# imatge-upc/rsis

Measured on AMD Instinct MI355X. Metric: training images/sec at 256x256, T=10, batch=32 per GPU, higher is better.
Workload: dtype f32

## Files before the change

rsis_amd/csrc/api.hip:

```cpp
#include "common.h"
#include "../../include/rsis_hip.h"
#include "launchers.h"
#include <stdlib.h>

static inline int krows_of(int C, int ks) { return rsis_roundup(C * ks * ks, RSIS_KPAD); }
static inline int log2i(int s) { int l = 0; while ((1 << l) < s) ++l; return l; }
static inline bool use_direct(int ks, int stride, int pad) { return ks == 3 && stride == 1 && pad == 1; }
static inline bool use_direct_s2(int ks, int stride, int pad) { return ks == 3 && stride == 2 && pad == 1; }
static inline bool use_direct_f2(int ks, int stride, int pad) {
  static const bool on = !(getenv("RSIS_CONV_F2") && getenv("RSIS_CONV_F2")[0] == '0');
  return on && use_direct_s2(ks, stride, pad);
}
static inline bool use_direct_fwd(int ks, int stride, int pad) { return use_direct(ks, stride, pad) || use_direct_f2(ks, stride, pad); }
static inline int seg_chunks(int nseg, const int* Cseg, int ck) {
  int q = 0;
  for (int s = 0; s < nseg; ++s) q += (Cseg[s] + ck - 1) / ck;
  return q;
}
static inline int direct_rows(int nseg, const int* Cseg) { return seg_chunks(nseg, Cseg, RSIS_CK) * RSIS_CK * 9; }
static inline bool bf16_geom(int ks, int stride, int pad, int Cout) {
  return Cout > 1 && ((ks == 3 && stride == 1 && pad == 1) || (ks == 1 && pad == 0));
}
static inline bool use_bf16(int dtype, int ks, int stride, int pad, int Cout) {
  return dtype == RSIS_DTYPE_BF16 && bf16_geom(ks, stride, pad, Cout);
}
static inline bool wino_geom(int ks, int stride, int pad, int Cin, int Cout, int nseg, int lstm_hid) {
  return ks == 3 && stride == 1 && pad == 1 && nseg == 1 && lstm_hid == 0 && Cin >= 32 && Cout >= 32 && Cin % 32 == 0 && Cout % 32 == 0;
}
static inline bool wino_geom_dgrad(int ks, int stride, int pad, int Cin, int Cout) {
  return ks == 3 && stride == 1 && pad == 1 && Cin >= 32 && Cout >= 32 && Cin % 32 == 0 && Cout % 32 == 0;
}
static inline bool use_wino(int dtype, int ks, int stride, int pad, int Cin, int Cout, int nseg, int lstm_hid) {
  return dtype == RSIS_DTYPE_F32_WINO && wino_geom(ks, stride, pad, Cin, Cout, nseg, lstm_hid);
}
static inline int bf16_rows(int ks, int nseg, const int* Cseg) {
  const int ckb = bf16_ckb(ks * ks);
  return seg_chunks(nseg, Cseg, ckb) * ks * ks * (ckb / 8);
}
static int g_deterministic = -1;
int rsis_deterministic() {
  if (g_deterministic < 0) g_deterministic = (getenv("RSIS_DETERMINISTIC") && getenv("RSIS_DETERMINISTIC")[0] == '1') ? 1 : 0;
  return g_deterministic;
}
static inline bool conv_splitk_ok() {
  static const bool env_ok = !(getenv("RSIS_CONV_SPLITK") && getenv("RSIS_CONV_SPLITK")[0] == '0');
  return env_ok && !rsis_deterministic();
}
static inline bool splitk_geom(int B, int H, int W, int rows, int nq, int min_chunks) {
  const long px_tiles = (long)B * rsis_cdiv(H, 8) * rsis_cdiv(W, W <= 8 ? 8 : 16);
  return nq >= min_chunks && px_tiles * rsis_cdiv(rows, 64) < 160;
}
static int zero_dsts(const ConvArgs& a, hipStream_t st) {
  for (int i = 0; i < a.ndst; ++i)
    if (rsis_zero_async(a.dst[i], sizeof(float) * (size_t)a.B * a.Cd[i] * a.oH * a.oW, st) != RSIS_OK) return RSIS_ERR_LAUNCH;
  return RSIS_OK;
}
static int splitk_enable(ConvArgs& a, hipStream_t st) { a.ksplit = 0; return zero_dsts(a, st); }
static inline int direct_variant(int tile) { const int v = tile % 10; return (tile > 0 && v >= 1 && v <= 9) ? v : 0; }

extern "C" {

int rsis_version(void) { return RSIS_ABI_VERSION; }

int rsis_set_deterministic(int on) {
// ... 179 lines not shown
  a.nsrc = nsrc;
  a.K = 0;
  for (int s = 0; s < RSIS_MAX_SRC; ++s) { a.src[s] = nsrc > 0 ? src[0] : nullptr; a.C[s] = 0; }
  for (int s = 0; s < nsrc; ++s) {
    if (!src[s] || Csrc[s] < 1) return RSIS_ERR_ARG;
    a.src[s] = src[s]; a.C[s] = Csrc[s]; a.K += Csrc[s] * ks * ks;
  }
  return RSIS_OK;
}

struct BnEval { const float* gamma; const float* beta; const float* mean; const float* var; float eps; int relu; };

static int conv2d_fwd_impl(const float* const* src, const int* Csrc, int nsrc, int B, int H, int W, const void* Wp, int Cout,
                           int ks, int stride, int pad, const float* bias, const float* addend, float* out, int Ho, int Wo,
                           int tile, int dtype, void* stream, const BnEval* bn) {
  const bool allow_splitk = tile >= 100;
  tile %= 100;
  ConvArgs a = {};
  int rc = fill_sources(a, src, Csrc, nsrc, ks);
  if (rc) return rc;
  if (!Wp || !out || B < 1 || stride < 1) return RSIS_ERR_ARG;
  if (Ho != (H + 2 * pad - ks) / stride + 1 || Wo != (W + 2 * pad - ks) / stride + 1) return RSIS_ERR_ARG;
  a.B = B; a.H = H; a.W = W; a.Ho = Ho; a.Wo = Wo; a.stride = stride; a.pad = pad; a.sshift = 0;
  a.wp = (const float*)Wp; a.ldw = rsis_roundup(Cout, RSIS_LDW_ALIGN); a.Cout = Cout; a.bias = bias; a.addend = addend;
  a.dst[0] = out; a.Cd[0] = Cout; a.ndst = 1;
  a.ostride = 1; a.oH = Ho; a.oW = Wo; a.ksplit = 1;
  a.precise = allow_splitk ? 0 : 1;
  if (bn) {
    if (!bn->gamma || !bn->beta || !bn->mean || !bn->var) return RSIS_ERR_ARG;
    if (allow_splitk || Cout % 4 != 0 || (size_t)B * Cout * Ho * Wo * 4 >= (1ull << 31)) return RSIS_ERR_UNSUPPORTED;
    if (dtype != RSIS_DTYPE_F32 && (dtype != RSIS_DTYPE_BF16 || use_bf16(dtype, ks, stride, pad, Cout))) return RSIS_ERR_UNSUPPORTED;
    if (use_direct(ks, stride, pad) && Cout == 1) return RSIS_ERR_UNSUPPORTED;
    a.ep_gamma = bn->gamma; a.ep_beta = bn->beta; a.ep_mean = bn->mean; a.ep_var = bn->var; a.ep_eps = bn->eps; a.ep_relu = bn->relu ? 1 : 0;
  }
  if (use_wino(dtype, ks, stride, pad, Csrc[0], Cout, nsrc, 0))
    return rsis_launch_conv_wino(src[0], Wp, bias, addend, out, B, Csrc[0], Cout, H, W, (hipStream_t)stream, a.precise);
  if (use_bf16(dtype, ks, stride, pad, Cout)) {
    if (stride != 1) return RSIS_ERR_UNSUPPORTED;
    if (ks == 1 && nsrc != 1) return RSIS_ERR_UNSUPPORTED;
    if (ks == 3 && allow_splitk && conv_splitk_ok() && !addend && splitk_geom(B, H, W, Cout, seg_chunks(a.nsrc, a.C, RSIS_CKB3), 16) &&
        splitk_enable(a, (hipStream_t)stream))
      return RSIS_ERR_LAUNCH;
    return rsis_launch_conv_bf16(a, ks, 0, direct_variant(tile), (hipStream_t)stream);
  }
  if (use_direct(ks, stride, pad) && Cout == 1 && nsrc == 1 && !addend && rsis_c1_supported(Csrc[0]) && W % 4 == 0)
    return rsis_l_c1_fwd(src[0], (const float*)Wp, a.ldw, bias, out, B, Csrc[0], H, W, 1, (hipStream_t)stream);
  if (use_direct(ks, stride, pad)) {
    if (allow_splitk && conv_splitk_ok() && splitk_geom(B, H, W, Cout, seg_chunks(a.nsrc, a.C, RSIS_CK), 32) && splitk_enable(a, (hipStream_t)stream))
      return RSIS_ERR_LAUNCH;
    return rsis_launch_conv3x3_direct(a, 0, direct_variant(tile), (hipStream_t)stream);
  }
  if (use_direct_f2(ks, stride, pad))
    return rsis_launch_conv3x3_direct(a, 3, direct_variant(tile), (hipStream_t)stream);
  return rsis_launch_conv_igemm(a, ks, false, 0, tile, (hipStream_t)stream);
}

int rsis_conv2d_fwd(const float* const* src, const int* Csrc, int nsrc, int B, int H, int W, const void* Wp, int Cout,
                    int ks, int stride, int pad, const float* bias, const float* addend, float* out, int Ho, int Wo,
                    int tile, int dtype, void* stream) {
  return conv2d_fwd_impl(src, Csrc, nsrc, B, H, W, Wp, Cout, ks, stride, pad, bias, addend, out, Ho, Wo, tile, dtype, stream, nullptr);
}

int rsis_conv2d_fwd_bn_eval(const float* const* src, const int* Csrc, int nsrc, int B, int H, int W, const void* Wp, int Cout,
                            int ks, int stride, int pad, const float* bias, const float* addend, const float* gamma, const float* beta,
                            const float* running_mean, const float* running_var, float eps, int relu, float* out, int Ho, int Wo,
                            int tile, int dtype, void* stream) {
  const BnEval bn = {gamma, beta, running_mean, running_var, eps, relu};
  return conv2d_fwd_impl(src, Csrc, nsrc, B, H, W, Wp, Cout, ks, stride, pad, bias, addend, out, Ho, Wo, tile % 100, dtype, stream, &bn);
}

static int dgrad_fill(ConvArgs& a, const float* dy, int B, int Cout, int Hy, int Wy, const void* Wd, int Cin_packed, int ks, int stride, int pad,
                      float* const* dx, const int* Cdx, int ndst, int Hx, int Wx, const float* addend) {
  a = ConvArgs{};
  const float* srcs[1] = {dy};
  const int cs[1] = {Cout};
  const int rc = fill_sources(a, srcs, cs, 1, ks);
  if (rc) return rc;
  int ctot = 0;
  for (int i = 0; i < ndst; ++i) { if (!dx[i] || Cdx[i] < 1) return RSIS_ERR_ARG; a.dst[i] = dx[i]; a.Cd[i] = Cdx[i]; ctot += Cdx[i]; }
  if (ctot > Cin_packed) return RSIS_ERR_ARG;
  a.ndst = ndst;
  a.B = B; a.H = Hy; a.W = Wy; a.Ho = Hx; a.Wo = Wx; a.stride = stride; a.pad = pad; a.sshift = log2i(stride);
  a.ostride = 1; a.oH = Hx; a.oW = Wx; a.ksplit = 1;
  a.wp = (const float*)Wd; a.ldw = rsis_roundup(Cin_packed, RSIS_LDW_ALIGN); a.Cout = ctot; a.bias = nullptr; a.addend = addend;
  return RSIS_OK;
}

int rsis_conv2d_dgrad(const float* dy, int B, int Cout, int Hy, int Wy, const void* Wd, int Cin_packed, int ks, int stride,
                      int pad, float* const* dx, const int* Cdx, int ndst, int Hx, int Wx, const float* addend, int tile,
                      int dtype, void* stream) {
  if (!dy || !Wd || !dx || !Cdx || ndst < 1 || ndst > RSIS_MAX_SRC) return RSIS_ERR_ARG;
  const bool inplace = addend && ndst == 1 && stride > 1 && ks == 1 && pad == 0 && addend == dx[0];
  if (addend && !inplace && (ndst != 1 || stride != 1)) return RSIS_ERR_UNSUPPORTED;
  if (stride != 1 && stride != 2 && stride != 4) return RSIS_ERR_UNSUPPORTED;
  ConvArgs a;
  const int rc = dgrad_fill(a, dy, B, Cout, Hy, Wy, Wd, Cin_packed, ks, stride, pad, dx, Cdx, ndst, Hx, Wx, addend);
  if (rc) return rc;
  const int ctot = a.Cout;
  if (dtype == RSIS_DTYPE_F32_WINO && wino_geom_dgrad(ks, stride, pad, Cin_packed, Cout)) {
    if (ndst > 2 || ctot % 32 != 0 || Cdx[0] % 32 != 0 || Hx != Hy || Wx != Wy || (ndst == 2 && addend)) return RSIS_ERR_UNSUPPORTED;
    if (ndst == 1) return rsis_launch_conv_wino(dy, Wd, nullptr, addend, dx[0], B, Cout, ctot, Hy, Wy, (hipStream_t)stream, 0);
    const float* xs[1] = {dy}; const void* us[1] = {Wd}; float* y0[1] = {dx[0]}; float* y1[1] = {dx[1]};
    const int b1[1] = {B}, c1[1] = {Cout}, co1[1] = {ctot}, c01[1] = {Cdx[0]}, h1[1] = {Hy}, w1[1] = {Wy};
    return rsis_launch_conv_wino_group(1, xs, us, y0, y1, b1, c1, co1, c01, h1, w1, (hipStream_t)stream);
  }
  if (use_bf16(dtype, ks, stride, pad, Cout)) {
    if (ks == 3) {
      if (Hx != Hy || Wx != Wy) return RSIS_ERR_ARG;
      if (conv_splitk_ok() && !addend && splitk_geom(B, Hx, Wx, ctot, seg_chunks(a.nsrc, a.C, RSIS_CKB3), 16) && splitk_enable(a, (hipStream_t)stream))
        return RSIS_ERR_LAUNCH;
      return rsis_launch_conv_bf16(a, 3, 0, direct_variant(tile), (hipStream_t)stream);
    }
    if (stride > 1) {
      if (Hy != (Hx - 1) / stride + 1 || Wy != (Wx - 1) / stride + 1) return RSIS_ERR_ARG;
      if (!inplace && zero_dsts(a, (hipStream_t)stream)) return RSIS_ERR_LAUNCH;
      a.ostride = stride;
    } else if (Hx != Hy || Wx != Wy) return RSIS_ERR_ARG;
    a.Ho = Hy; a.Wo = Wy; a.stride = 1; a.sshift = 0;
    return rsis_launch_conv_bf16(a, 1, 0, direct_variant(tile), (hipStream_t)stream);
  }
  if (use_direct(ks, stride, pad)) {
    if (Hx != Hy || Wx != Wy) return RSIS_ERR_ARG;
    if (Cout == 1 && ndst == 1 && Cin_packed == Cdx[0] && rsis_c1_supported(Cdx[0]) && !addend)
      return rsis_l_c1_dgrad(dy, (const float*)Wd, a.ldw, dx[0], B, Cdx[0], Hx, Wx, 1, (hipStream_t)stream);
    if (conv_splitk_ok() && !addend && splitk_geom(B, Hx, Wx, ctot, seg_chunks(a.nsrc, a.C, RSIS_CK), 32) && splitk_enable(a, (hipStream_t)stream))
      return RSIS_ERR_LAUNCH;
    return rsis_launch_conv3x3_direct(a, 0, direct_variant(tile), (hipStream_t)stream);
  }
  if (use_direct_s2(ks, stride, pad) && ndst == 1 && Cdx[0] == Cin_packed && Hy == (Hx + 1) / 2 && Wy == (Wx + 1) / 2) {
    a.Ho = Hy; a.Wo = Wy; a.oH = Hx; a.oW = Wx;
    return rsis_launch_conv3x3_direct(a, 2, direct_variant(tile), (hipStream_t)stream);
  }
  if (ks == 1 && pad == 0 && stride > 1) {
    if (!inplace && zero_dsts(a, (hipStream_t)stream)) return RSIS_ERR_LAUNCH;
    a.Ho = Hy; a.Wo = Wy; a.stride = 1; a.sshift = 0; a.ostride = stride;
    return rsis_launch_conv_igemm(a, ks, false, 0, tile, (hipStream_t)stream);
  }
  return rsis_launch_conv_igemm(a, ks, true, 0, tile, (hipStream_t)stream);
}

static int wgrad_route(WgradArgs& a, int ks, int lstm_hid, int dtype) {
  if (dtype == RSIS_DTYPE_BF16_BLK) {
    a.blk = 1;
    return rsis_wgrad_bf16_supported(a, ks) ? 1 : -1;
  }
  if (use_direct(ks, a.stride, a.pad) && a.Cout == 1 && lstm_hid == 0 && rsis_c1_supported(a.Cs) && a.H == a.Ho && a.W == a.Wo && a.W % 4 == 0)
    return 0;
  if (dtype == RSIS_DTYPE_BF16 && rsis_wgrad_bf16_supported(a, ks)) return 1;
  static const bool tiled_ok = !(getenv("RSIS_WGRAD_TILED") && getenv("RSIS_WGRAD_TILED")[0] == '0');
  if (tiled_ok && rsis_wgrad_tiled_supported(a, ks)) return 2;
  return 3;
}
static int wgrad_fill(WgradArgs& a, const float* dy, const float* x, float* dW, int B, int Cs, int H, int W, int Cout, int Ho, int Wo,
                      int ks, int stride, int pad, int Ctot, int c_off, int lstm_hid) {
  if (!dy || !x || !dW || c_off < 0 || c_off + Cs > Ctot) return RSIS_ERR_ARG;
  a = WgradArgs{};
  a.dy = dy; a.x = x; a.dw = dW; a.B = B; a.Cs = Cs; a.H = H; a.W = W; a.Ho = Ho; a.Wo = Wo; a.Cout = Cout;
  a.stride = stride; a.pad = pad; a.ldo = Ctot * ks * ks; a.n_off = c_off * ks * ks; a.interleave_hid = lstm_hid;
  return RSIS_OK;
}
static int wgrad_launch_one(WgradArgs& a, int route, int ks, hipStream_t st) {
  switch (route) {
    case 0: return rsis_l_c1_wgrad(a.dy, a.x, a.dw + a.n_off, nullptr, a.B, a.Cs, a.H, a.W, 1, st);
    case 1: return rsis_launch_conv_wgrad_bf16(a, ks, st);
    case 2: return rsis_launch_conv_wgrad_tiled(a, ks, st);
    default: return rsis_launch_conv_wgrad(a, ks, st);
  }
}

int rsis_conv2d_wgrad(const float* dy, const float* x, float* dW, int B, int Cs, int H, int W, int Cout, int Ho, int Wo,
                      int ks, int stride, int pad, int Ctot, int c_off, int lstm_hid, int dtype, void* stream) {
  WgradArgs a;
  const int rc = wgrad_fill(a, dy, x, dW, B, Cs, H, W, Cout, Ho, Wo, ks, stride, pad, Ctot, c_off, lstm_hid);
  if (rc) return rc;
  const int route = wgrad_route(a, ks, lstm_hid, dtype);
  if (route < 0) return RSIS_ERR_UNSUPPORTED;
  return wgrad_launch_one(a, route, ks, (hipStream_t)stream);
}

int rsis_conv2d_wgrad_batch(const rsis_wgrad_job* jobs, int njobs, void* stream) {
  if (!jobs || njobs < 1) return RSIS_ERR_ARG;
  WgradArgs* tiled[4] = {(WgradArgs*)malloc(sizeof(WgradArgs) * njobs), (WgradArgs*)malloc(sizeof(WgradArgs) * njobs),
                         (WgradArgs*)malloc(sizeof(WgradArgs) * njobs), (WgradArgs*)malloc(sizeof(WgradArgs) * njobs)};
  int nt[4] = {0, 0, 0, 0};
  int rc = (tiled[0] && tiled[1] && tiled[2] && tiled[3]) ? RSIS_OK : RSIS_ERR_LAUNCH;
  for (int j = 0; j < njobs && rc == RSIS_OK; ++j) {
    const rsis_wgrad_job& q = jobs[j];
    WgradArgs a;
    rc = wgrad_fill(a, q.dy, q.x, q.dW, q.B, q.Cs, q.H, q.W, q.Cout, q.Ho, q.Wo, q.ks, q.stride, q.pad, q.Ctot, q.c_off, q.lstm_hid);
    if (rc) break;
    const int route = wgrad_route(a, q.ks, q.lstm_hid, q.dtype);
    if (route < 0) { rc = RSIS_ERR_UNSUPPORTED; break; }
    if ((route == 1 || route == 2) && (q.ks == 1 || q.ks == 3) && !rsis_deterministic()) {
      const int li = (route == 1 ? 2 : 0) + (q.ks == 3);
      tiled[li][nt[li]++] = a;
    } else rc = wgrad_launch_one(a, route, q.ks, (hipStream_t)stream);
  }
  if (rc == RSIS_OK) rc = rsis_launch_conv_wgrad_tiled_group(tiled[0], nt[0], 1, (hipStream_t)stream);
  if (rc == RSIS_OK) rc = rsis_launch_conv_wgrad_tiled_group(tiled[1], nt[1], 3, (hipStream_t)stream);
  if (rc == RSIS_OK) rc = rsis_launch_conv_wgrad_bf16_group(tiled[2], nt[2], 1, (hipStream_t)stream);
  if (rc == RSIS_OK) rc = rsis_launch_conv_wgrad_bf16_group(tiled[3], nt[3], 3, (hipStream_t)stream);
  for (int i = 0; i < 4; ++i) free(tiled[i]);
  return rc;
}

int rsis_bias_grad(const float* dy, float* db, int B, int C, int HW, int lstm_hid, void* stream) {
  if (!dy || !db) return RSIS_ERR_ARG;
  return rsis_l_channel_sum(dy, db, B, C, HW, lstm_hid, (hipStream_t)stream);
}

static int lstm_fill(ConvArgs& a, int& route, const float* const* src, const int* Csrc, int nsrc, int B, int H, int W, const void* Wp,
                     const float* bias_packed, const float* addend, const float* c_prev, float* h_out, float* c_out, float* act_out, int hid,
                     int ks, int pad, int dtype, unsigned long long* side_key = nullptr) {
  a = ConvArgs{};
  int rc = fill_sources(a, src, Csrc, nsrc, ks, addend != nullptr);
  if (rc) return rc;
  if (!Wp || !h_out || !c_out || hid < 1 || B < 1) return RSIS_ERR_ARG;
  if (2 * pad != ks - 1) return RSIS_ERR_UNSUPPORTED;
// ... 564 lines not shown
```

rsis_amd/csrc/launchers.h:

```cpp
#pragma once
#include "common.h"
#include "../../include/rsis_hip.h"

int rsis_launch_conv_igemm(ConvArgs& a, int ks, bool dgrad, int epi, int force_tile, hipStream_t st);
int rsis_launch_conv3x3_direct(ConvArgs& a, int epi, int force_variant, hipStream_t st);
int rsis_launch_convlstm_direct_group(ConvArgs* jobs, int n, const int* force_variant, hipStream_t st);
int rsis_launch_conv3x3_direct_group_plain(ConvArgs* jobs, int n, const int* force_variant, hipStream_t st);
int rsis_launch_conv_wino(const float* x, const void* U, const float* bias, const float* addend, float* y, int B, int C, int Cout, int H, int W, hipStream_t st,
                          int precise);
int rsis_launch_conv_wino_group(int n, const float* const* x, const void* const* U, float* const* y, float* const* y1, const int* B, const int* C, const int* Cout,
                                const int* C0, const int* H, const int* W, hipStream_t st);
int rsis_launch_conv_bf16(ConvArgs& a, int ks, int epi, int force_variant, hipStream_t st);
int rsis_launch_conv_blk(ConvArgs& a, int ks, int variant, hipStream_t st);
int rsis_l_blk_from_nchw(const float* x, void* y, int B, int C, int HW, hipStream_t st);
int rsis_l_blk_to_nchw(const void* x, float* y, int B, int C, int HW, hipStream_t st);
int rsis_launch_conv_blk_dec(BlkConvJob* jobs, int n, int epi, const int* force_variant, hipStream_t st);
int rsis_launch_conv_wgrad(WgradArgs& a, int ks, hipStream_t st);
bool rsis_wgrad_bf16_supported(const WgradArgs& w, int ks);
int rsis_launch_conv_wgrad_bf16_group(const WgradArgs* w, int n, int ks, hipStream_t st);
int rsis_launch_conv_wgrad_bf16(const WgradArgs& w, int ks, hipStream_t st);
int rsis_launch_conv_wgrad_tiled_group(const WgradArgs* w, int n, int ks, hipStream_t st);
int rsis_launch_conv_wgrad_tiled(const WgradArgs& w, int ks, hipStream_t st);
bool rsis_wgrad_tiled_supported(const WgradArgs& w, int ks);
bool rsis_c1_supported(int Cin);
int rsis_l_c1_fwd(const float* x, const float* wp, int ldw, const float* bias, float* y, int B, int Cin, int H, int W, int seqT, hipStream_t st);
int rsis_l_c1_dgrad(const float* dy, const float* wd, int ldw, float* dx, int B, int Cin, int H, int W, int seqT, hipStream_t st);
int rsis_l_c1_wgrad(const float* dy, const float* x, float* dw, float* db, int B, int Cin, int H, int W, int seqT, hipStream_t st);
bool rsis_upconv_supported(int C, int Hs, int Ws, int Ho, int Wo);
int rsis_upconv_bwd_blocks(int T, int B, int Hs, int Ws);
int rsis_l_upconv_fwd(const void* h, int h_blk, const float* w, const float* bias, float* out, int T, int B, int Hs, int Ws, int Ho, int Wo, hipStream_t st);
int rsis_l_upconv_bwd(const float* dout, const void* h, int h_blk, const float* w, void* dh, float* dW, float* db, const float* dside, const int* arg,
                      float* partial, int T, int B, int Hs, int Ws, int Ho, int Wo, hipStream_t st);
int rsis_l_pack_batch(const rsis_pack_job* jobs, int njobs, int total_blocks, hipStream_t st);
int rsis_l_pack_blocks(PackMode mode, int krows, int ldw, int ks);
int rsis_l_pack(PackMode mode, const float* W, void* out, int Cout, int Ctot, int ks, int nseg, const int* Cseg, const int* Coff, int ldw, int krows, int hid,
                hipStream_t st);
int rsis_l_lstm_bwd(const float* dh, const float* dh2, const float* dc_next, const float* act, const float* c_prev, const float* c, float* da, float* dc_prev,
                    float* da_sum, int B, int hid, int HW, hipStream_t st);
int rsis_l_lstm_bwd_group(const void* const* ptrs, const int* dims, int n, hipStream_t st);
int rsis_l_upsample_fwd(const float* x, float* y, long BC, int Hi, int Wi, int Ho, int Wo, hipStream_t st);
int rsis_l_upsample_bwd(const float* dy, float* dx, long BC, int Hi, int Wi, int Ho, int Wo, const float* pool_g, const int* pool_arg, hipStream_t st);
int rsis_l_gmax_fwd(const float* x, float* y, int* arg, long BC, int HW, hipStream_t st);
int rsis_l_gmax_bwd(const float* dy, const int* arg, float* dx, long BC, int HW, hipStream_t st);
int rsis_l_bn_fwd(const float* x, const float* res, float* y, unsigned char* mask, double* stats, const float* gamma, const float* beta, float* run_mean,
                  float* run_var, float* save_mean, float* save_rstd, int B, int C, int HW, float eps, float momentum, int relu, int train_flags, hipStream_t st);
int rsis_l_bn_bwd(const float* dy, const float* x, const float* y, const unsigned char* mask, const float* mean, const float* rstd, const float* gamma,
                  double* stats, float* dx, float* dres, float* dgamma, float* dbeta, int B, int C, int HW, int relu_flags, float eval_eps, hipStream_t st);
int rsis_l_gmax_bwd_add(const float* dy, const int* arg, float* dx, long BC, int HW, hipStream_t st);
int rsis_l_subsample(const float* x, float* y, long BC, int H, int W, int Ho, int Wo, int s, hipStream_t st);
int rsis_l_maxpool_fwd(const float* x, float* y, unsigned char* arg, long BC, int H, int W, int Ho, int Wo, hipStream_t st);
int rsis_l_maxpool_bwd(const float* dy, const unsigned char* arg, float* dx, long BC, int H, int W, int Ho, int Wo, int accumulate, hipStream_t st);
int rsis_l_sum_leading(const float* x, float* y, int T, long n, hipStream_t st);
int rsis_l_channel_sum(const float* dy, float* db, int B, int C, int HW, int hid, hipStream_t st);
int rsis_l_adam(float* p, const float* g, float* m, float* v, long n, float lr, float b1, float b2, float eps, float wd, int step, float gscale, const int* step_dev,
                hipStream_t st);
int rsis_l_assign(const float* scores, long long* perm, int B, int G, int T, hipStream_t st);
int rsis_l_flat_rule(int rule, float* p, const float* g, float* s, long n, float lr, float c0, float c1, float wd, float gscale, hipStream_t st);
// ... 64 lines not shown
```

rsis_amd/csrc/pointwise.hip:

```cpp
#include "common.h"
#include "launchers.h"
#include <cstdlib>

__global__ void lstm_bwd_kernel(const float* __restrict__ dh, const float* __restrict__ dh2, const float* __restrict__ dc_next,
                                const float* __restrict__ act, const float* __restrict__ c_prev,
                                const float* __restrict__ c, float* __restrict__ da, float* __restrict__ dc_prev,
                                float* __restrict__ da_sum, int hid, int HW, long total) {
  for (long e = blockIdx.x * (long)blockDim.x + threadIdx.x; e < total; e += (long)gridDim.x * blockDim.x) {
    const long bj = e / HW;
    const int sp = (int)(e - bj * HW);
    const long g0 = bj * 4 * HW + sp;
    const float gi = act[g0], gf = act[g0 + HW], go = act[g0 + 2L * HW], gg = act[g0 + 3L * HW];
    const float tc = tanhf(c[e]);
    const float dhv = (dh ? dh[e] : 0.f) + (dh2 ? dh2[e] : 0.f);
    float dcv = dhv * go * (1.f - tc * tc);
    if (dc_next) dcv += dc_next[e];
    const float cp = c_prev ? c_prev[e] : 0.f;
    const float dai = dcv * gg * gi * (1.f - gi);
    const float daf = dcv * cp * gf * (1.f - gf);
    const float dao = dhv * tc * go * (1.f - go);
    const float dag = dcv * gi * (1.f - gg * gg);
    da[g0] = dai; da[g0 + HW] = daf; da[g0 + 2L * HW] = dao; da[g0 + 3L * HW] = dag;
    if (da_sum) { da_sum[g0] += dai; da_sum[g0 + HW] += daf; da_sum[g0 + 2L * HW] += dao; da_sum[g0 + 3L * HW] += dag; }
    if (dc_prev) dc_prev[e] = dcv * gf;
// ... 661 lines not shown
      const size_t idx = ((size_t)b * C + c) * HW + sp;
      f32x4 o;
#pragma unroll
      for (int k = 0; k < 4; ++k) o[k] = kk * (g[i][k] - mg - xh[i][k] * mgx);
      *reinterpret_cast<f32x4*>(dx + idx) = o;
      if (dres) *reinterpret_cast<f32x4*>(dres + idx) = g[i];
    }
  }
}

__global__ void subsample_kernel(const float* __restrict__ x, float* __restrict__ y, int H, int W, int Ho, int Wo, int s, long total4) {
  const int wq = (Wo + 3) / 4;
  for (long e = blockIdx.x * (long)blockDim.x + threadIdx.x; e < total4; e += (long)gridDim.x * blockDim.x) {
    const int q = (int)(e % wq);
    const long t = e / wq;
    const int ho = (int)(t % Ho);
    const long bc = t / Ho;
    const float* xr = x + (bc * H + (long)ho * s) * W;
    float* yr = y + (bc * Ho + ho) * (long)Wo + 4 * q;
    if (s == 2 && (W & 3) == 0 && 4 * q + 3 < Wo && 8 * q + 7 < W) {
      const f32x4 a = *reinterpret_cast<const f32x4*>(xr + 8 * q), b = *reinterpret_cast<const f32x4*>(xr + 8 * q + 4);
      const f32x4 o = {a[0], a[2], b[0], b[2]};
      if ((Wo & 3) == 0) *reinterpret_cast<f32x4*>(yr) = o;
      else { yr[0] = o[0]; yr[1] = o[1]; yr[2] = o[2]; yr[3] = o[3]; }
    } else {
      for (int k = 0; k < 4 && 4 * q + k < Wo; ++k) yr[k] = xr[(long)(4 * q + k) * s];
    }
  }
}

__global__ void maxpool3x3s2_fwd_kernel(const float* __restrict__ x, float* __restrict__ y, unsigned char* __restrict__ arg,
                                        int H, int W, int Ho, int Wo, long total) {
  for (long e = blockIdx.x * (long)blockDim.x + threadIdx.x; e < total; e += (long)gridDim.x * blockDim.x) {
    const int wo = (int)(e % Wo);
    const long t = e / Wo;
    const int ho = (int)(t % Ho);
    const long bc = t / Ho;
    const float* xb = x + bc * H * W;
    float v[9];
    bool ok[9];
#pragma unroll
    for (int r = 0; r < 3; ++r)
#pragma unroll
      for (int s = 0; s < 3; ++s) {
        const int h = ho * 2 - 1 + r, w = wo * 2 - 1 + s;
        ok[r * 3 + s] = (unsigned)h < (unsigned)H && (unsigned)w < (unsigned)W;
        v[r * 3 + s] = xb[min(max(h, 0), H - 1) * W + min(max(w, 0), W - 1)];
      }
    float best = -INFINITY; int bi = 0;
#pragma unroll
    for (int k = 0; k < 9; ++k)
      if (ok[k] && (v[k] > best || v[k] != v[k])) { best = v[k]; bi = k; }
    y[e] = best; arg[e] = (unsigned char)bi;
  }
}

__global__ void maxpool3x3s2_bwd_kernel(const float* __restrict__ dy, const unsigned char* __restrict__ arg,
                                        float* __restrict__ dx, int H, int W, int Ho, int Wo, long total, int accumulate) {
  for (long e = blockIdx.x * (long)blockDim.x + threadIdx.x; e < total; e += (long)gridDim.x * blockDim.x) {
    const int w = (int)(e % W);
    const long t = e / W;
    const int h = (int)(t % H);
    const long bc = t / H;
    float g = 0.f;
    const int ho_lo = h >> 1, wo_lo = w >> 1;
#pragma unroll
    for (int a = 0; a < 2; ++a) {
#pragma unroll
      for (int b = 0; b < 2; ++b) {
        const int ho = ho_lo + a, wo = wo_lo + b;
        const int r = h - (ho * 2 - 1), s = w - (wo * 2 - 1);
        const bool ok = ho < Ho && r >= 0 && r <= 2 && wo < Wo && s >= 0 && s <= 2;
        const long o = (bc * Ho + min(ho, Ho - 1)) * Wo + min(wo, Wo - 1);
        const int ar = arg[o];
        const float d = dy[o];
        g += (ok && ar == r * 3 + s) ? d : 0.f;
      }
    }
    if (accumulate) g += dx[e];
    dx[e] = g;
  }
}

__global__ __launch_bounds__(256) void maxpool3x3s2_bwd_v8_kernel(const float* __restrict__ dy, const unsigned char* __restrict__ arg,
                                                                  float* __restrict__ dx, int H, int W, int Ho, int Wo, long items,
                                                                  int accumulate) {
  const int Wq = W >> 2, Hp = H >> 1;
  for (long e = blockIdx.x * (long)blockDim.x + threadIdx.x; e < items; e += (long)gridDim.x * blockDim.x) {
    const int wq = (int)(e % Wq);
    const long t = e / Wq;
    const int hp = (int)(t % Hp);
    const long bc = t / Hp;
    const int h0 = hp * 2, w0 = wq * 4;
    float d[6];
    int th[6], tw[6];
#pragma unroll
    for (int a = 0; a < 2; ++a)
#pragma unroll
      for (int b = 0; b < 3; ++b) {
        const int ho = hp + a, wo = wq * 2 + b;
        const bool ok = ho < Ho && wo < Wo;
        const long o = (bc * Ho + min(ho, Ho - 1)) * Wo + min(wo, Wo - 1);
        const int ar = arg[o];
        d[a * 3 + b] = dy[o];
        th[a * 3 + b] = ok ? ho * 2 - 1 + ar / 3 - h0 : -1;
        tw[a * 3 + b] = wo * 2 - 1 + ar % 3 - w0;
// ... 377 lines not shown
}
template <int NT, int VPT>
static void bn_bwd_fused_launch(const float* dy, const float* x, const float* y, const unsigned char* mask, const float* mean,
                                const float* rstd, const float* gamma, float* dx, float* dres, float* dgamma, float* dbeta, int C,
                                int HW, long N, int relu, int accum, hipStream_t st) {
  if (mask)
    hipLaunchKernelGGL((bn_bwd_fused_kernel<NT, VPT, true>), dim3(C), dim3(NT), 0, st, dy, x, y, mask, mean, rstd, gamma, dx, dres,
                       dgamma, dbeta, C, HW, N, relu, accum);
  else
    hipLaunchKernelGGL((bn_bwd_fused_kernel<NT, VPT, false>), dim3(C), dim3(NT), 0, st, dy, x, y, mask, mean, rstd, gamma, dx, dres,
                       dgamma, dbeta, C, HW, N, relu, accum);
}
int rsis_l_bn_bwd(const float* dy, const float* x, const float* y, const unsigned char* mask, const float* mean, const float* rstd,
                  const float* gamma, double* stats, float* dx, float* dres, float* dgamma, float* dbeta, int B, int C, int HW,
                  int relu_flags, float eval_eps, hipStream_t st) {
  const long N = (long)B * HW;
  const int S = chan_splits(C, N);
  const int relu = relu_flags & 1, accum = (relu_flags >> 2) & 1;
  if (mask && (!relu || (HW & 3))) return RSIS_ERR_UNSUPPORTED;
  if (eval_eps < 0.f && bn_fused_ok(C, HW, N)) {
    if (N / 4 <= 256 * 8 && C <= 512)
      bn_bwd_fused_launch<512, 4>(dy, x, y, mask, mean, rstd, gamma, dx, dres, dgamma, dbeta, C, HW, N, relu, accum, st);
    else if (N / 4 <= 256 * 8)
      bn_bwd_fused_launch<256, 8>(dy, x, y, mask, mean, rstd, gamma, dx, dres, dgamma, dbeta, C, HW, N, relu, accum, st);
    else
      bn_bwd_fused_launch<1024, 8>(dy, x, y, mask, mean, rstd, gamma, dx, dres, dgamma, dbeta, C, HW, N, relu, accum, st);
    return rsis_check_launch();
  }
  if (!(relu_flags & 2) && rsis_zero_async(stats, sizeof(double) * 2 * C, st) != RSIS_OK) return RSIS_ERR_LAUNCH;
  if (mask) {
    hipLaunchKernelGGL(bn_bwd_reduce_kernel<true>, dim3(C, S), dim3(256), 0, st, dy, x, y, mask, mean, rstd, stats, C, HW, N, relu,
                       eval_eps);
    hipLaunchKernelGGL(bn_bwd_apply_kernel<true>, dim3(C, S), dim3(256), 0, st, dy, x, y, mask, mean, rstd, gamma, stats, dx, dres,
                       dgamma, dbeta, C, HW, N, relu, accum, eval_eps);
  } else {
    hipLaunchKernelGGL(bn_bwd_reduce_kernel<false>, dim3(C, S), dim3(256), 0, st, dy, x, y, mask, mean, rstd, stats, C, HW, N, relu,
                       eval_eps);
    hipLaunchKernelGGL(bn_bwd_apply_kernel<false>, dim3(C, S), dim3(256), 0, st, dy, x, y, mask, mean, rstd, gamma, stats, dx, dres,
                       dgamma, dbeta, C, HW, N, relu, accum, eval_eps);
  }
  return rsis_check_launch();
}
int rsis_l_gmax_bwd_add(const float* dy, const int* arg, float* dx, long BC, int HW, hipStream_t st) {
  hipLaunchKernelGGL(global_maxpool_bwd_add_kernel, dim3((unsigned)((BC + 255) / 256)), dim3(256), 0, st, dy, arg, dx, HW, BC);
  return rsis_check_launch();
}
int rsis_l_subsample(const float* x, float* y, long BC, int H, int W, int Ho, int Wo, int s, hipStream_t st) {
  const long total4 = BC * Ho * ((Wo + 3) / 4);
  hipLaunchKernelGGL(subsample_kernel, dim3(ew_grid(total4)), dim3(256), 0, st, x, y, H, W, Ho, Wo, s, total4);
  return rsis_check_launch();
}
int rsis_l_maxpool_fwd(const float* x, float* y, unsigned char* arg, long BC, int H, int W, int Ho, int Wo, hipStream_t st) {
  const long total = BC * Ho * Wo;
  hipLaunchKernelGGL(maxpool3x3s2_fwd_kernel, dim3(ew_grid(total)), dim3(256), 0, st, x, y, arg, H, W, Ho, Wo, total);
  return rsis_check_launch();
}
int rsis_l_maxpool_bwd(const float* dy, const unsigned char* arg, float* dx, long BC, int H, int W, int Ho, int Wo, int accumulate,
                       hipStream_t st) {
  const long total = BC * H * W;
  if ((H & 1) == 0 && (W & 3) == 0) {
    hipLaunchKernelGGL(maxpool3x3s2_bwd_v8_kernel, dim3(ew_grid(total / 8)), dim3(256), 0, st, dy, arg, dx, H, W, Ho, Wo, total / 8,
                       accumulate);
    return rsis_check_launch();
  }
  hipLaunchKernelGGL(maxpool3x3s2_bwd_kernel, dim3(ew_grid(total)), dim3(256), 0, st, dy, arg, dx, H, W, Ho, Wo, total, accumulate);
  return rsis_check_launch();
}
__global__ __launch_bounds__(256) void sum_leading_kernel(const float* __restrict__ x, float* __restrict__ y, int T, long n, long n4) {
  const long e = (long)blockIdx.x * 256 + threadIdx.x;
  if (e < n4) {
    const f32x4* p = reinterpret_cast<const f32x4*>(x) + e;
    f32x4 acc = p[0];
    for (int t = 1; t < T; ++t) { const f32x4 v = p[(size_t)t * (n / 4)]; acc[0] += v[0]; acc[1] += v[1]; acc[2] += v[2]; acc[3] += v[3]; }
    reinterpret_cast<f32x4*>(y)[e] = acc;
  } else {
    const long i = 4 * n4 + (e - n4);
    if (i < n) { float acc = x[i]; for (int t = 1; t < T; ++t) acc += x[(size_t)t * n + i]; y[i] = acc; }
  }
}
int rsis_l_sum_leading(const float* x, float* y, int T, long n, hipStream_t st) {
  const bool v4 = (n % 4 == 0) && ((((size_t)x | (size_t)y) & 15) == 0);
  const long n4 = v4 ? n / 4 : 0, threads = n4 + (n - 4 * n4);
  hipLaunchKernelGGL(sum_leading_kernel, dim3((unsigned)((threads + 255) / 256)), dim3(256), 0, st, x, y, T, n, n4);
  return rsis_check_launch();
}

int rsis_l_channel_sum(const float* dy, float* db, int B, int C, int HW, int hid, hipStream_t st) {
  const long N = (long)B * HW;
  int S = chan_splits(C, N);
  if (S > 512) S = 512;
  hipLaunchKernelGGL(channel_sum_kernel, dim3(C, S), dim3(256), 0, st, dy, db, C, HW, N, hid);
  return rsis_check_launch();
}
int rsis_l_adam(float* p, const float* g, float* m, float* v, long n, float lr, float b1, float b2, float eps, float wd,
                int step, float gscale, const int* step_dev, hipStream_t st) {
  hipLaunchKernelGGL(adam_kernel, dim3(ew_grid(n)), dim3(256), 0, st, p, g, m, v, n, lr, b1, b2, eps, wd, step, gscale, step_dev);
  return rsis_check_launch();
}

int rsis_l_assign(const float* scores, long long* perm, int B, int G, int T, hipStream_t st) {
  if (G > RSIS_ASSIGN_MAX2) return RSIS_ERR_ARG;
  if (G <= RSIS_ASSIGN_MAX) hipLaunchKernelGGL(assign_kernel, dim3(B), dim3(64), 0, st, scores, perm, B, G, T);
  else hipLaunchKernelGGL(assign2_kernel, dim3(B), dim3(64), sizeof(float) * (size_t)G * (T < 2 ? 2 : T), st, scores, perm, B, G, T);
  return rsis_check_launch();
}
```

Baseline: 958.9.

## Add MFMA-based 7x7 stride-2 stem conv kernels and vectorized maxpool forward

Adds dedicated kernels for the 3-channel 7x7 stride-2 stem convolution. The forward kernel stages the weights and a parity-split input patch in LDS through buffer-to-LDS loads, then runs fp32 32x32x2 MFMA, replacing the generic implicit-GEMM path. The weight-gradient kernel is persistent and double-buffers input patches, accumulating the result with atomicAdd, so it is skipped in deterministic mode. A 4-wide vectorized 3x3 stride-2 maxpool forward is also added. All three are enabled by default behind environment switches.

Result: no change. 967.2 (median of 6 runs) (+0.9%).

```diff
diff --git a/rsis_amd/csrc/api.hip b/rsis_amd/csrc/api.hip
--- a/rsis_amd/csrc/api.hip
+++ b/rsis_amd/csrc/api.hip
@@ -10,6 +10,10 @@
 static inline bool use_direct_f2(int ks, int stride, int pad) {
   static const bool on = !(getenv("RSIS_CONV_F2") && getenv("RSIS_CONV_F2")[0] == '0');
   return on && use_direct_s2(ks, stride, pad);
+}
+static inline bool stem_on() {
+  static const bool on = !(getenv("RSIS_STEM") && getenv("RSIS_STEM")[0] == '0');
+  return on;
 }
 static inline bool use_direct_fwd(int ks, int stride, int pad) { return use_direct(ks, stride, pad) || use_direct_f2(ks, stride, pad); }
 static inline int seg_chunks(int nseg, const int* Cseg, int ck) {
@@ -295,6 +299,7 @@
   }
   if (use_direct_f2(ks, stride, pad))
     return rsis_launch_conv3x3_direct(a, 3, direct_variant(tile), (hipStream_t)stream);
+  if (allow_splitk && tile == 0 && !bn && stem_on() && rsis_conv_stem_fwd_supported(a, ks)) return rsis_launch_conv_stem_fwd(a, (hipStream_t)stream);
   return rsis_launch_conv_igemm(a, ks, false, 0, tile, (hipStream_t)stream);
 }
 
@@ -390,6 +395,7 @@
   if (use_direct(ks, a.stride, a.pad) && a.Cout == 1 && lstm_hid == 0 && rsis_c1_supported(a.Cs) && a.H == a.Ho && a.W == a.Wo && a.W % 4 == 0)
     return 0;
   if (dtype == RSIS_DTYPE_BF16 && rsis_wgrad_bf16_supported(a, ks)) return 1;
+  if (stem_on() && !rsis_deterministic() && lstm_hid == 0 && rsis_conv_stem_wgrad_supported(a, ks)) return 4;
   static const bool tiled_ok = !(getenv("RSIS_WGRAD_TILED") && getenv("RSIS_WGRAD_TILED")[0] == '0');
   if (tiled_ok && rsis_wgrad_tiled_supported(a, ks)) return 2;
   return 3;
@@ -407,6 +413,7 @@
     case 0: return rsis_l_c1_wgrad(a.dy, a.x, a.dw + a.n_off, nullptr, a.B, a.Cs, a.H, a.W, 1, st);
     case 1: return rsis_launch_conv_wgrad_bf16(a, ks, st);
     case 2: return rsis_launch_conv_wgrad_tiled(a, ks, st);
+    case 4: return rsis_launch_conv_stem_wgrad(a, st);
     default: return rsis_launch_conv_wgrad(a, ks, st);
   }
 }
diff --git a/rsis_amd/csrc/conv_stem.hip b/rsis_amd/csrc/conv_stem.hip
--- /dev/null
+++ b/rsis_amd/csrc/conv_stem.hip
@@ -0,0 +1,287 @@
+#include "common.h"
+#include "launchers.h"
+
+#define ST_TH 8
+#define ST_TW 32
+#define ST_PR (2 * ST_TH + 5)
+#define ST_PH 36
+#define ST_PROW (2 * ST_PH)
+#define ST_PCH (ST_PR * ST_PROW)
+#define ST_PATCH (3 * ST_PCH)
+#define ST_PLOADS 18
+#define ST_K 148
+#define ST_WLDS (ST_K * 64)
+#define ST_WF4 (ST_WLDS / 4)
+#define ST_WLOADS ((ST_WF4 + 255) / 256)
+#define ST_OOB 0x7FFFFFF0u
+
+typedef __attribute__((address_space(3))) void* st_lds_vp_t;
+typedef const float __attribute__((address_space(1)))* st_gcf_t;
+
+__host__ __device__ constexpr int st_poff(int k) {
+  return (k / 49) * ST_PCH + ((k % 49) / 7) * ST_PROW + (((k % 49) % 7) & 1) * ST_PH + (((k % 49) % 7) >> 1);
+}
+__host__ __device__ constexpr int st_delta(int kk) { return 2 * kk + 1 >= 147 ? 36 : st_poff(2 * kk + 1) - st_poff(2 * kk); }
+static_assert(st_delta(0) == 36 && st_delta(4) == -35 && st_delta(3) == 69 && st_delta(24) == 1077, "tap distances");
+
+__global__ __launch_bounds__(256) void conv_stem_fwd_kernel(const ConvArgs p, const int tiles_x, const int tiles_y) {
+#if __HIP_DEVICE_COMPILE__
+  __shared__ __attribute__((aligned(16))) float lds[ST_WLDS + ST_PLOADS * 256];
+  float* const Ws = lds;
+  float* const Ps = lds + ST_WLDS;
+
+  const int tid = threadIdx.x, lane = tid & 63, l31 = lane & 31, hi = lane >> 5;
+  const int wave = __builtin_amdgcn_readfirstlane(tid >> 6);
+  const int H = p.H, W = p.W, Ho = p.Ho, Wo = p.Wo, HW = H * W, HoWo = Ho * Wo, Cout = p.Cout;
+  const int bid = blockIdx.x;
+  const int tx = bid % tiles_x, t2 = bid / tiles_x;
+  const int ty = t2 % tiles_y, img = t2 / tiles_y;
+  const int ho0 = ty * ST_TH, wo0 = tx * ST_TW;
+
+  {
+    const __amdgpu_buffer_rsrc_t rw = __builtin_amdgcn_make_buffer_rsrc((void*)p.wp, 0, 147 * p.ldw * 4, 0x00020000);
+#pragma unroll
+    for (int i = 0; i < ST_WLOADS; ++i) {
+      const int idx = tid + i * 256;
+      if (i * 256 + wave * 64 < ST_WF4)
+        __builtin_amdgcn_raw_ptr_buffer_load_lds(rw, (st_lds_vp_t)(Ws + i * 1024 + wave * 256), 16, (unsigned)((idx >> 4) * p.ldw + (idx & 15) * 4) * 4u, 0, 0, 0);
+    }
+  }
+  {
+    const __amdgpu_buffer_rsrc_t rx = __builtin_amdgcn_make_buffer_rsrc((void*)(p.src[0] + (size_t)img * 3 * HW), 0, 3 * HW * 4, 0x00020000);
+    const int gy0 = 2 * ho0 - 3, gx0 = 2 * wo0 - 3;
+#pragma unroll
+    for (int i = 0; i < ST_PLOADS; ++i) {
+      const int e = tid + i * 256;
+      const int ci = e / ST_PCH, rem = e - ci * ST_PCH;
+      const int row = rem / ST_PROW, q = rem - row * ST_PROW;
+      const int par = q >= ST_PH ? 1 : 0;
+      const int c = 2 * (q - par * ST_PH) + par;
+      const int gy = gy0 + row, gx = gx0 + c;
+      const bool ok = e < ST_PATCH && c < 2 * ST_TW + 5 && (unsigned)gy < (unsigned)H && (unsigned)gx < (unsigned)W;
+      __builtin_amdgcn_raw_ptr_buffer_load_lds(rx, (st_lds_vp_t)(Ps + i * 256 + wave * 64), 4, ok ? (unsigned)(ci * HW + gy * W + gx) * 4u : ST_OOB, 0, 0, 0);
+    }
+  }
+
+  f32x16 acc[2][2];
+#pragma unroll
+  for (int i = 0; i < 2; ++i)
+#pragma unroll
+    for (int j = 0; j < 2; ++j)
+#pragma unroll
+      for (int r = 0; r < 16; ++r) acc[i][j][r] = 0.f;
+
+  __builtin_amdgcn_s_waitcnt(0x0F70);
+  __syncthreads();
+
+  const float* const wa = Ws + hi * 64 + l31;
+  const float* const pb = Ps + (4 * wave) * ST_PROW + l31;
+  const float* const pb0 = pb + hi * 36;
+  const float* const pb1 = pb - hi * 35;
+  const float* const pb2 = pb + hi * 69;
+  const float* const pb3 = pb + hi * 1077;
+#pragma unroll
+  for (int kk = 0; kk < ST_K / 2; ++kk) {
+    const int d = st_delta(kk), o = st_poff(2 * kk);
+    const float* const bp = d == 36 ? pb0 : (d == -35 ? pb1 : (d == 69 ? pb2 : pb3));
+    const float a0 = wa[kk * 128], a1 = wa[kk * 128 + 32];
+    float b0 = bp[o], b1 = bp[o + 2 * ST_PROW];
+    if (2 * kk + 1 >= 147) { b0 = hi ? 0.f : b0; b1 = hi ? 0.f : b1; }
+    acc[0][0] = __builtin_amdgcn_mfma_f32_32x32x2f32(a0, b0, acc[0][0], 0, 0, 0);
+    acc[0][1] = __builtin_amdgcn_mfma_f32_32x32x2f32(a0, b1, acc[0][1], 0, 0, 0);
+    acc[1][0] = __builtin_amdgcn_mfma_f32_32x32x2f32(a1, b0, acc[1][0], 0, 0, 0);
+    acc[1][1] = __builtin_amdgcn_mfma_f32_32x32x2f32(a1, b1, acc[1][1], 0, 0, 0);
+  }
+
+  const st_gcf_t bias = (st_gcf_t)p.bias;
+  const __amdgpu_buffer_rsrc_t ro = __builtin_amdgcn_make_buffer_rsrc((void*)p.dst[0], 0, (unsigned)((size_t)p.B * Cout * HoWo * 4), 0x00020000);
+  const unsigned rowb = (unsigned)HoWo * 4u;
+  const int wo = wo0 + l31;
+#pragma unroll
+  for (int j = 0; j < 2; ++j) {
+    const int ho = ho0 + 2 * wave + j;
+    const bool pxv = ho < Ho && wo < Wo;
+#pragma unroll
+    for (int i = 0; i < 2; ++i) {
+      const int row0 = i * 32 + 4 * hi;
+      const unsigned vo = (unsigned)((img * Cout + row0) * HoWo + ho * Wo + wo) * 4u;
+      const int rows_left = pxv ? Cout - row0 : 0;
+#pragma unroll
+      for (int r = 0; r < 16; ++r) {
+        const int k = (r & 3) + 8 * (r >> 2);
+        float v = acc[i][j][r];
+        if (bias) v += k < rows_left ? bias[row0 + k] : 0.f;
+        __builtin_amdgcn_raw_buffer_store_b32(__builtin_bit_cast(unsigned, v), ro, k < rows_left ? vo + k * rowb : ST_OOB, 0, 0);
+      }
+    }
+  }
+#endif
+}
+
+#define SW_TH 4
+#define SW_PR (2 * SW_TH + 5)
+#define SW_PROW 71
+#define SW_PCH (SW_PR * SW_PROW)
+#define SW_PATCH (3 * SW_PCH)
+#define SW_PLOADS 11
+#define SW_PX (SW_TH * ST_TW)
+#define SW_DYLDS (SW_PX * 64)
+
+template <int NB>
+__device__ __forceinline__ void sw_tile(f32x16 (&acc)[3], const float* ap, const float* b0, const float* b1, const float* b2) {
+  const float* const bs[3] = {b0, b1, b2};
+#pragma unroll
+  for (int kk = 0; kk < SW_PX / 2; ++kk) {
+    const int o = (kk >> 4) * 2 * SW_PROW + (kk & 15) * 2;
+    const float a = ap[kk * 128];
+#pragma unroll
+    for (int j = 0; j < NB; ++j) acc[j] = __builtin_amdgcn_mfma_f32_32x32x2f32(a, bs[j][o], acc[j], 0, 0, 0);
+  }
+}
+
+template <bool V4>
+__global__ __launch_bounds__(256) void conv_stem_wgrad_kernel(const WgradArgs p, const int tiles_x, const int tiles_y, const int n_tiles) {
+#if __HIP_DEVICE_COMPILE__
+  __shared__ __attribute__((aligned(16))) float lds[SW_DYLDS + 2 * SW_PLOADS * 256];
+  float* const Dy = lds;
+  float* const Ps0 = lds + SW_DYLDS;
+
+  const int tid = threadIdx.x, lane = tid & 63, l31 = lane & 31, hi = lane >> 5;
+  const int wave = __builtin_amdgcn_readfirstlane(tid >> 6);
+  const int H = p.H, W = p.W, Ho = p.Ho, Wo = p.Wo, HW = H * W, Cout = p.Cout;
+  const int wm = wave >> 1, wn = (wave ^ (int)(blockIdx.x >> 8)) & 1;
+  const int t_begin = (int)((long)blockIdx.x * n_tiles / gridDim.x), t_end = (int)((long)(blockIdx.x + 1) * n_tiles / gridDim.x);
+
+  int noff[3];
+#pragma unroll
+  for (int j = 0; j < 3; ++j) {
+    const int n = min((wn * 3 + j) * 32 + l31, 146);
+    const int ci = n / 49, rs = n - ci * 49, r = rs / 7, s = rs - r * 7;
+    noff[j] = ci * SW_PCH + r * SW_PROW + (s & 1) * 36 + (s >> 1) + hi;
+  }
+  const int s_co = tid & 63, s_q = tid >> 6;
+  f32x4 dreg[8];
+
+  auto tile_origin = [&](int t, int& img, int& ho0, int& wo0) {
+    const int tx = t % tiles_x, t2 = t / tiles_x;
+    wo0 = tx * ST_TW; ho0 = (t2 % tiles_y) * SW_TH; img = t2 / tiles_y;
+  };
+  auto issue_patch = [&](int t, int buf) {
+    int img, ho0, wo0;
+    tile_origin(t, img, ho0, wo0);
+    const __amdgpu_buffer_rsrc_t rx = __builtin_amdgcn_make_buffer_rsrc((void*)(p.x + (size_t)img * 3 * HW), 0, 3 * HW * 4, 0x00020000);
+    const int gy0 = 2 * ho0 - 3, gx0 = 2 * wo0 - 3;
+    float* const Ps = Ps0 + buf * (SW_PLOADS * 256);
+#pragma unroll
+    for (int i = 0; i < SW_PLOADS; ++i) {
+      const int e = tid + i * 256;
+      const int ci = e / SW_PCH, rem = e - ci * SW_PCH;
+      const int row = rem / SW_PROW, q = rem - row * SW_PROW;
+      const int par = q >= 36 ? 1 : 0;
+      const int c = 2 * (q - par * 36) + par;
+      const int gy = gy0 + row, gx = gx0 + c;
+      const bool ok = e < SW_PATCH && c < 2 * ST_TW + 5 && (unsigned)gy < (unsigned)H && (unsigned)gx < (unsigned)W;
+      __builtin_amdgcn_raw_ptr_buffer_load_lds(rx, (st_lds_vp_t)(Ps + i * 256 + wave * 64), 4, ok ? (unsigned)(ci * HW + gy * W + gx) * 4u : ST_OOB, 0, 0, 0);
+    }
+  };
+  auto load_dy = [&](int t) {
+    int img, ho0, wo0;
+    tile_origin(t, img, ho0, wo0);
+#pragma unroll
+    for (int it = 0; it < 8; ++it) {
+      const int q = s_q * 8 + it;
+      const int ho = ho0 + (q >> 3), wo = wo0 + (q & 7) * 4;
+      const float* g = p.dy + (((size_t)img * Cout + s_co) * Ho + ho) * Wo + wo;
+      const bool ok = s_co < Cout && ho < Ho;
+      f32x4 v = {0.f, 0.f, 0.f, 0.f};
+      if constexpr (V4) {
+        if (ok && wo < Wo) v = *reinterpret_cast<const f32x4*>(g);
+      } else {
+#pragma unroll
+        for (int k = 0; k < 4; ++k)
+          if (ok && wo + k < Wo) v[k] = g[k];
+      }
+      dreg[it] = v;
+    }
+  };
+  auto store_dy = [&]() {
+#pragma unroll
+    for (int it = 0; it < 8; ++it) {
+      const int q = s_q * 8 + it;
+      float* d = Dy + ((q >> 3) * ST_TW + (q & 7) * 4) * 64 + s_co;
+#pragma unroll
+      for (int k = 0; k < 4; ++k) d[k * 64] = dreg[it][k];
+    }
+  };
+
+  f32x16 acc[3];
+#pragma unroll
+  for (int j = 0; j < 3; ++j)
+#pragma unroll
+    for (int r = 0; r < 16; ++r) acc[j][r] = 0.f;
+
+  if (t_begin < t_end) {
+    issue_patch(t_begin, 0);
+    load_dy(t_begin);
+  }
+  const float* const ap = Dy + hi * 64 + wm * 32 + l31;
+  for (int t = t_begin; t < t_end; ++t) {
+    const int buf = (t - t_begin) & 1;
+    __builtin_amdgcn_s_waitcnt(0x0F70);
+    store_dy();
+    __syncthreads();
+    if (t + 1 < t_end) {
+      issue_patch(t + 1, buf ^ 1);
+      load_dy(t + 1);
+    }
+    const float* const Ps = Ps0 + buf * (SW_PLOADS * 256);
+    const float* const b0 = Ps + noff[0], * const b1 = Ps + noff[1], * const b2 = Ps + noff[2];
+    if (wn == 0) sw_tile<3>(acc, ap, b0, b1, b2);
+    else sw_tile<2>(acc, ap, b0, b1, b2);
+    __syncthreads();
+  }
+
+  if (t_begin < t_end) {
+#pragma unroll
+    for (int j = 0; j < 3; ++j) {
+      const int n = (wn * 3 + j) * 32 + l31;
+      if (n >= 147 || (wn == 1 && j == 2)) continue;
+#pragma unroll
+      for (int r = 0; r < 16; ++r) {
+        const int co = wm * 32 + (r & 3) + 8 * (r >> 2) + 4 * hi;
+        if (co < Cout) atomicAdd(p.dw + (size_t)co * p.ldo + p.n_off + n, acc[j][r]);
+      }
+    }
+  }
+#endif
+}
+
+bool rsis_conv_stem_wgrad_supported(const WgradArgs& a, int ks) {
+  return ks == 7 && a.stride == 2 && a.pad == 3 && a.Cs == 3 && a.Cout >= 1 && a.Cout <= 64 && a.interleave_hid == 0 && !a.blk &&
+         a.Ho == (a.H - 1) / 2 + 1 && a.Wo == (a.W - 1) / 2 + 1 && (long)3 * a.H * a.W * 4 < (1L << 31);
+}
+
+int rsis_launch_conv_stem_wgrad(const WgradArgs& a, hipStream_t st) {
+  const int tiles_x = rsis_cdiv(a.Wo, ST_TW), tiles_y = rsis_cdiv(a.Ho, SW_TH);
+  const long n_tiles = (long)a.B * tiles_y * tiles_x;
+  if (n_tiles < 1 || n_tiles >= (1L << 31)) return RSIS_ERR_UNSUPPORTED;
+  const int grid = (int)(n_tiles < 512 ? n_tiles : 512);
+  if (a.Wo % 4 == 0 && ((uintptr_t)a.dy & 15) == 0)
+    hipLaunchKernelGGL(conv_stem_wgrad_kernel<true>, dim3(grid), dim3(256), 0, st, a, tiles_x, tiles_y, (int)n_tiles);
+  else
+    hipLaunchKernelGGL(conv_stem_wgrad_kernel<false>, dim3(grid), dim3(256), 0, st, a, tiles_x, tiles_y, (int)n_tiles);
+  return rsis_check_launch();
+}
+
+bool rsis_conv_stem_fwd_supported(const ConvArgs& a, int ks) {
+  return ks == 7 && a.stride == 2 && a.pad == 3 && a.nsrc == 1 && a.C[0] == 3 && a.Cout >= 1 && a.Cout <= 64 && !a.addend && !a.ep_gamma && a.ndst == 1 &&
+         (long)3 * a.H * a.W * 4 < (1L << 31) && (long)a.B * a.Cout * a.Ho * a.Wo * 4 < (1L << 31);
+}
+
+int rsis_launch_conv_stem_fwd(const ConvArgs& a, hipStream_t st) {
+  const int tiles_x = rsis_cdiv(a.Wo, ST_TW), tiles_y = rsis_cdiv(a.Ho, ST_TH);
+  const long grid = (long)a.B * tiles_y * tiles_x;
+  if (grid < 1 || grid >= (1L << 31)) return RSIS_ERR_UNSUPPORTED;
+  hipLaunchKernelGGL(conv_stem_fwd_kernel, dim3((unsigned)grid), dim3(256), 0, st, a, tiles_x, tiles_y);
+  return rsis_check_launch();
+}
diff --git a/rsis_amd/csrc/launchers.h b/rsis_amd/csrc/launchers.h
--- a/rsis_amd/csrc/launchers.h
+++ b/rsis_amd/csrc/launchers.h
@@ -3,6 +3,10 @@
 #include "../../include/rsis_hip.h"
 
 int rsis_launch_conv_igemm(ConvArgs& a, int ks, bool dgrad, int epi, int force_tile, hipStream_t st);
+bool rsis_conv_stem_fwd_supported(const ConvArgs& a, int ks);
+int rsis_launch_conv_stem_fwd(const ConvArgs& a, hipStream_t st);
+bool rsis_conv_stem_wgrad_supported(const WgradArgs& a, int ks);
+int rsis_launch_conv_stem_wgrad(const WgradArgs& a, hipStream_t st);
 int rsis_launch_conv3x3_direct(ConvArgs& a, int epi, int force_variant, hipStream_t st);
 int rsis_launch_convlstm_direct_group(ConvArgs* jobs, int n, const int* force_variant, hipStream_t st);
 int rsis_launch_conv3x3_direct_group_plain(ConvArgs* jobs, int n, const int* force_variant, hipStream_t st);
diff --git a/rsis_amd/csrc/pointwise.hip b/rsis_amd/csrc/pointwise.hip
--- a/rsis_amd/csrc/pointwise.hip
+++ b/rsis_amd/csrc/pointwise.hip
@@ -737,6 +737,48 @@
     for (int k = 0; k < 9; ++k)
       if (ok[k] && (v[k] > best || v[k] != v[k])) { best = v[k]; bi = k; }
     y[e] = best; arg[e] = (unsigned char)bi;
+  }
+}
+
+__global__ __launch_bounds__(256) void maxpool3x3s2_fwd_v4_kernel(const float* __restrict__ x, float* __restrict__ y,
+                                                                  unsigned char* __restrict__ arg, int H, int W, int Ho, int Wo, long items) {
+  const int Wq = Wo >> 2;
+  for (long e = blockIdx.x * (long)blockDim.x + threadIdx.x; e < items; e += (long)gridDim.x * blockDim.x) {
+    const int q = (int)(e % Wq);
+    const long t = e / Wq;
+    const int ho = (int)(t % Ho);
+    const long bc = t / Ho;
+    const float* xb = x + bc * H * W;
+    float v[3][9];
+    bool okr[3];
+#pragma unroll
+    for (int r = 0; r < 3; ++r) {
+      const int h = ho * 2 - 1 + r;
+      okr[r] = (unsigned)h < (unsigned)H;
+      const float* xr = xb + (long)min(max(h, 0), H - 1) * W + 8 * q;
+      const f32x4 a = *reinterpret_cast<const f32x4*>(xr), b = *reinterpret_cast<const f32x4*>(xr + 4);
+      v[r][0] = xr[q > 0 ? -1 : 0];
+      v[r][1] = a[0]; v[r][2] = a[1]; v[r][3] = a[2]; v[r][4] = a[3];
+      v[r][5] = b[0]; v[r][6] = b[1]; v[r][7] = b[2]; v[r][8] = b[3];
+    }
+    f32x4 o;
+    unsigned ab = 0;
+#pragma unroll
+    for (int k = 0; k < 4; ++k) {
+      float best = -INFINITY; int bi = 0;
+#pragma unroll
+      for (int r = 0; r < 3; ++r)
+#pragma unroll
+        for (int s = 0; s < 3; ++s) {
+          const bool ok = okr[r] && (s > 0 || k > 0 || q > 0);
+          const float c = v[r][2 * k + s];
+          if (ok && (c > best || c != c)) { best = c; bi = r * 3 + s; }
+        }
+      o[k] = best; ab |= (unsigned)bi << (8 * k);
+    }
+    const long ob = (bc * Ho + ho) * Wo + 4 * q;
+    *reinterpret_cast<f32x4*>(y + ob) = o;
+    *reinterpret_cast<unsigned*>(arg + ob) = ab;
   }
 }
 
@@ -1220,6 +1262,11 @@
 }
 int rsis_l_maxpool_fwd(const float* x, float* y, unsigned char* arg, long BC, int H, int W, int Ho, int Wo, hipStream_t st) {
   const long total = BC * Ho * Wo;
+  static const bool v4_on = !(getenv("RSIS_MAXPOOL_V4") && getenv("RSIS_MAXPOOL_V4")[0] == '0');
+  if (v4_on && (W & 7) == 0 && Wo == W / 2 && Ho == (H - 1) / 2 + 1 && (((uintptr_t)x | (uintptr_t)y) & 15) == 0 && ((uintptr_t)arg & 3) == 0) {
+    hipLaunchKernelGGL(maxpool3x3s2_fwd_v4_kernel, dim3(ew_grid(total / 4)), dim3(256), 0, st, x, y, arg, H, W, Ho, Wo, total / 4);
+    return rsis_check_launch();
+  }
   hipLaunchKernelGGL(maxpool3x3s2_fwd_kernel, dim3(ew_grid(total)), dim3(256), 0, st, x, y, arg, H, W, Ho, Wo, total);
   return rsis_check_launch();
 }
```
